# daducci/AMICO

Measured on AMD Instinct MI355X. Metric: voxels/sec (whole node), NODDI fit, higher is better.
Workload: dtype f64; 1 GPU; NODDI fit, 1000000 masked voxels per GPU, 99-volume 2-shell scheme (9 b0 + 30@b700 + 60@b2000), 145 atoms, ndirs=500, inputs resident in HBM; voxels_per_gpu=1000000, global_voxels=1000000, parallelism=voxel shards x1, one RCCL all_gather of the maps per step

## Files before the change

amico_amd/csrc/amx_seed.hpp:

```cpp
#pragma once
#include "amx_kernels.hpp"

namespace amx {

constexpr int kSeedMax = 8;
constexpr int kSeed3ListRow = 36;
constexpr int kSeed3ScanMax = 32;
constexpr int kStageUbNorm = 2;
constexpr int kStageUb = 4;
template <int KD, int LD, int UB = kStageUb>
__device__ __forceinline__ void stage_rows(double *Sl, const double *__restrict__ Sg, int n, int src_ld)
{
    const int N = n * KD;
    for (int e0 = threadIdx.x; e0 < N; e0 += UB * (int)blockDim.x) {
        double v[UB];
#pragma unroll
        for (int u = 0; u < UB; u++) {
            const int e = e0 + u * (int)blockDim.x, ec = e < N ? e : 0, j = ec / KD, d = ec - j * KD;
            v[u] = Sg[(size_t)j * src_ld + d];
        }
#pragma unroll
        for (int u = 0; u < UB; u++) {
            const int e = e0 + u * (int)blockDim.x, j = e / KD, d = e - j * KD;
            if (e < N) Sl[j * LD + d] = v[u];
// ... 74 lines not shown
            int bj = 0; double bn = red[0];
            for (int j = 1; j < n_cols && j < nt; j++) if (red[j] > bn) { bn = red[j]; bj = j; }
            s_j = bj; s_n = bn;
        }
        __syncthreads();
        const double nn = s_n;
        const bool live = nn > 1e-280;
        for (int i = tid; i < nS; i += nt) Q[d * nS + i] = live ? R[i * ldA + s_j] / sqrt(nn) : 0.0;
        __syncthreads();
        for (int pass = 0; pass < 2 && live; pass++) {
            if (tid < d) { double c = 0.0; for (int i = 0; i < nS; i++) c += Q[tid * nS + i] * Q[d * nS + i]; s_coef[tid] = c; }
            __syncthreads();
            for (int i = tid; i < nS; i += nt) { double v = Q[d * nS + i]; for (int e = 0; e < d; e++) v -= s_coef[e] * Q[e * nS + i]; Q[d * nS + i] = v; }
            __syncthreads();
            if (tid == 0) { double c = 0.0; for (int i = 0; i < nS; i++) c += Q[d * nS + i] * Q[d * nS + i]; s_n = c; }
            __syncthreads();
            const double n2 = s_n;
            for (int i = tid; i < nS; i += nt) Q[d * nS + i] = n2 > 0.0 ? Q[d * nS + i] / sqrt(n2) : 0.0;
            __syncthreads();
        }
        if (tid < n_cols) {
            double c = 0.0;
            for (int i = 0; i < nS; i++) c += Q[d * nS + i] * R[i * ldA + tid];
            for (int i = 0; i < nS; i++) R[i * ldA + tid] -= c * Q[d * nS + i];
        }
        __syncthreads();
    }
    if (kap != nullptr) {
        double en = 0.0, an = 0.0;
        if (tid < n_cols) {
            for (int i = 0; i < nS; i++) {
                const double v = R[i * ldA + tid]; en += v * v;
                double o = (rowsel == nullptr || rowsel[i]) ? (double)g[i * ldA + tid] : 0.0;
                if (colscale != nullptr) o *= colscale[tid];
                an += o * o;
            }
        }
        red[tid] = en;
        __syncthreads();
        if (tid == 0) { double m = 0.0; for (int j = 0; j < n_cols && j < nt; j++) m = red[j] > m ? red[j] : m; s_n = m; }
        __syncthreads();
        const double emax = sqrt(s_n);
        __syncthreads();
        red[tid] = an;
        __syncthreads();
        if (tid == 0) { double m = 0.0; for (int j = 0; j < n_cols && j < nt; j++) m = red[j] > m ? red[j] : m; kap[dir] = emax + 2e-6 * sqrt(m); if (kap0) kap0[dir] = emax; }
        __syncthreads();
    }
    double *U = Ub + (size_t)dir * nS * KD;
    for (int e = tid; e < nS * KD; e += nt) { const int i = e / KD, d = e - i * KD; U[e] = Q[d * nS + i]; }
    double *S = Sb + (size_t)dir * n_cols * KD;
    for (int e = tid; e < n_cols * KD; e += nt) {
        const int j = e / KD, d = e - j * KD;
        double c = 0.0;
        for (int i = 0; i < nS; i++) {
            double v = (rowsel == nullptr || rowsel[i]) ? (double)g[i * ldA + j] : 0.0;
            c += Q[d * nS + i] * v;
        }
        if (colscale != nullptr) c *= colscale[j];
        S[e] = c;
        if (Sf != nullptr) Sf[(size_t)dir * KD * kScreenLd + d * kScreenLd + j] = (float)c;
    }
}

struct SeedArgs {
    const double *y;
    const float *y32;
    const int *perm;
    const Chunk *chunks;
    const int *n_chunks;
    const Chunk *schunks;
    const int *n_schunks;
    const double *Ub, *Sb;
    double *ytil;
    unsigned long long *seeds;
    const unsigned long long *cand8; const unsigned char *cdone;
    const unsigned long long *supp;
    int nS, n_atoms, iso_atom, dot_atom;
    int *gcount;
    int n_gcount;
    int *stats;
    int trip_cap;
    int fork_skip;
};

template <int NR>
__global__ void __launch_bounds__(1024) k_noddi_project(const SeedArgs a)
{
    constexpr int KD = kSeedKD;
    const int cid = xcd_chunk((int)blockIdx.x, *a.n_chunks);
    if (cid < 0) return;
    const Chunk ck = a.chunks[cid];
    const int lane = threadIdx.x & 63, wave = threadIdx.x >> 6, nw = (int)blockDim.x >> 6;
    const int nS = a.nS;
    double ur[NR][KD];
    const double *U = a.Ub + (size_t)ck.dir * nS * KD;
#pragma unroll
    for (int rr = 0; rr < NR; rr++) {
        const int i = lane + kWave * rr;
#pragma unroll
        for (int d = 0; d < KD; d++) ur[rr][d] = (i < nS) ? U[i * KD + d] : 0.0;
    }
    for (int k = wave; k < ck.count; k += nw) {
        const int pos = ck.start + k;
        const size_t yo = (size_t)a.perm[pos] * nS;
        double yr[NR];
#pragma unroll
        for (int rr = 0; rr < NR; rr++) { const int i = lane + kWave * rr; yr[rr] = (i < nS) ? (a.y32 ? (double)a.y32[yo + i] : a.y[yo + i]) : 0.0; }
        double out = 0.0;
#pragma unroll
        for (int b = 0; b < KD; b += 4) {
            double p[4];
#pragma unroll
            for (int u = 0; u < 4; u++) {
                p[u] = 0.0;
#pragma unroll
                for (int rr = 0; rr < NR; rr++) p[u] += ur[rr][b + u] * yr[rr];
            }
            wave_sum4(p, lane);
#pragma unroll
            for (int u = 0; u < 4; u++) out = (lane == b + u) ? p[u] : out;
        }
        if (lane < KD) a.ytil[(size_t)pos * KD + lane] = out;
    }
}

__device__ __forceinline__ double seed_div(double x, double d)
{
    double r = __builtin_amdgcn_rcp(d);
    r = r * (2.0 - d * r);
    r = r * (2.0 - d * r);
    const double q = x * r;
    return q + r * (x - q * d);
}

template <int N> __device__ __forceinline__ constexpr int stri(int i, int j) { return i * (i + 1) / 2 + j; }


__device__ __forceinline__ double seed_max(double a, double b)
{
    double d;
    asm("v_max_f64 %0, %1, %2" : "=v"(d) : "v"(a), "v"(b));
    return d;
}

__device__ __forceinline__ double seed_min(double a, double b)
{
    double d;
    asm("v_min_f64 %0, %1, %2" : "=v"(d) : "v"(a), "v"(b));
    return d;
}

typedef double seed_v4d __attribute__((ext_vector_type(4)));
template <int KS, int MT, bool PIPE = true>
__device__ __forceinline__ void seed_scan_mfma(const double *Aop, double *Rb, const double (&r)[4 * KS], int lane, double &best, int &bj)
{
    constexpr int KDP = 4 * KS + 1;
    const int q = lane >> 4, c16 = lane & 15;
#pragma unroll
    for (int d = 0; d < 4 * KS; d++) Rb[lane * KDP + d] = r[d];
    double b[4][KS];
#pragma unroll
    for (int nt = 0; nt < 4; nt++) {
#pragma unroll
        for (int ks = 0; ks < KS; ks++) b[nt][ks] = Rb[(16 * nt + c16) * KDP + 4 * ks + q];
    }
    const double ninf = -__builtin_huge_val();
    double bv[4] = {ninf, ninf, ninf, ninf};
    auto products = [&](int mt, seed_v4d (&acc)[4]) {
        double av[KS];
#pragma unroll
        for (int ks = 0; ks < KS; ks++) av[ks] = Aop[(mt * KS + ks) * 64 + lane];
#pragma unroll
        for (int nt = 0; nt < 4; nt++) acc[nt] = (seed_v4d){0.0, 0.0, 0.0, 0.0};
#pragma unroll
        for (int ks = 0; ks < KS; ks++) {
#pragma unroll
            for (int nt = 0; nt < 4; nt++) acc[nt] = __builtin_amdgcn_mfma_f64_16x16x4f64(av[ks], b[nt][ks], acc[nt], 0, 0, 0);
        }
    };
    seed_v4d cur[4], nxt[PIPE ? 4 : 1];
    if (PIPE) products(0, cur);
#pragma unroll
    for (int mt = 0; mt < MT; mt++) {
        if (PIPE) { if (mt + 1 < MT) products(mt + 1, reinterpret_cast<seed_v4d (&)[4]>(nxt)); }
        else products(mt, cur);
        __builtin_amdgcn_sched_barrier(0);
#pragma unroll
        for (int nt = 0; nt < 4; nt++) {
#pragma unroll
            for (int rr = 0; rr < 4; rr++) {
                const double v = cur[nt][rr];
                const unsigned lo = ((unsigned)__double2loint(v) & 0xffffff00u) | (unsigned)(mt * 4 + rr);
                bv[nt] = seed_max(bv[nt], __hiloint2double(__double2hiint(v), (int)lo));
            }
        }
        __builtin_amdgcn_sched_barrier(0);
        if (PIPE) {
#pragma unroll
            for (int nt = 0; nt < 4; nt++) cur[nt] = nxt[PIPE ? nt : 0];
        }
    }
    double mine = ninf;
#pragma unroll
    for (int nt = 0; nt < 4; nt++) {
        const double t = __hiloint2double(__double2hiint(bv[nt]), (int)((unsigned)__double2loint(bv[nt]) | (unsigned)(q << 6)));
        const double m = rows_allmax(t);
        mine = (q == nt) ? m : mine;
    }
    const unsigned code = (unsigned)__double2loint(mine) & 0xffu;
    best = mine;
    bj = 16 * (int)((code >> 2) & 15u) + 4 * (int)(code & 3u) + (int)(code >> 6);
}

template <int MS>
struct SeedLane {
    static constexpr int NT = MS * (MS + 1) / 2;
    double T[NT], dinv[MS], c[MS], x[MS];
    int idx[MS], np;

    __device__ __forceinline__ void clear()
    {
        np = 0;
#pragma unroll
        for (int s = 0; s < MS; s++) { idx[s] = 0; x[s] = 0.0; c[s] = 0.0; dinv[s] = 0.0; }
#pragma unroll
        for (int e = 0; e < NT; e++) T[e] = 0.0;
    }
    __device__ __forceinline__ void solve(double (&z)[MS]) const
    {
#pragma unroll
        for (int j = 0; j < MS; j++) {
            double f = c[j];
#pragma unroll
            for (int m = 0; m < j; m++) f -= T[stri<MS>(j, m)] * z[m];
            z[j] = f * dinv[j];
        }
#pragma unroll
        for (int j = MS - 1; j >= 0; j--) {
            double f = z[j];
#pragma unroll
            for (int m = j + 1; m < MS; m++) f -= T[stri<MS>(m, j)] * z[m];
            z[j] = f * dinv[j];
        }
    }
    __device__ __forceinline__ void solve_rhs(const double (&b)[MS], double (&z)[MS]) const
    {
#pragma unroll
        for (int j = 0; j < MS; j++) {
            double f = b[j];
#pragma unroll
            for (int m = 0; m < j; m++) f -= T[stri<MS>(j, m)] * z[m];
            z[j] = f * dinv[j];
        }
#pragma unroll
        for (int j = MS - 1; j >= 0; j--) {
            double f = z[j];
#pragma unroll
            for (int m = j + 1; m < MS; m++) f -= T[stri<MS>(m, j)] * z[m];
            z[j] = f * dinv[j];
        }
    }
    __device__ __forceinline__ bool factor()
    {
        bool ok = true;
#pragma unroll
        for (int j = 0; j < MS; j++) {
            double dj = T[stri<MS>(j, j)];
            const double hjj = dj;
#pragma unroll
            for (int m = 0; m < j; m++) dj -= T[stri<MS>(j, m)] * T[stri<MS>(j, m)];
            const bool good = dj > 1e-15 * hjj;
            ok = ok && (j >= np || good);
            dinv[j] = (j < np && good) ? inv_sqrt(dj) : 0.0;
            T[stri<MS>(j, j)] = dj * dinv[j];
#pragma unroll
            for (int i = j + 1; i < MS; i++) {
                double v = T[stri<MS>(i, j)];
#pragma unroll
                for (int m = 0; m < j; m++) v -= T[stri<MS>(i, m)] * T[stri<MS>(j, m)];
                T[stri<MS>(i, j)] = v * dinv[j];
            }
        }
        return ok;
    }
    __device__ __forceinline__ void remove(int k)
    {
        double l[MS];
#pragma unroll
        for (int i = 0; i < MS - 1; i++) {
            double v = 0.0;
#pragma unroll
            for (int kk = 0; kk <= i; kk++) v = (k == kk) ? T[stri<MS>(i + 1, kk)] : v;
            l[i] = v;
        }
        l[MS - 1] = 0.0;
        __builtin_amdgcn_sched_barrier(0);
#pragma unroll
        for (int i = 0; i < MS - 1; i++) {
#pragma unroll
            for (int j = 0; j <= i; j++) {
                const double v00 = T[stri<MS>(i, j)], v10 = T[stri<MS>(i + 1, j)], v11 = T[stri<MS>(i + 1, j + 1)];
                T[stri<MS>(i, j)] = (i < k) ? v00 : ((j < k) ? v10 : v11);
            }
            __builtin_amdgcn_sched_barrier(0);
        }
        __builtin_amdgcn_sched_barrier(0);
#pragma unroll
        for (int m = 0; m < MS; m++) T[stri<MS>(MS - 1, m)] = (k < MS) ? 0.0 : T[stri<MS>(MS - 1, m)];
#pragma unroll
        for (int s = 0; s < MS - 1; s++) {
            const bool mv = s >= k;
            idx[s] = mv ? idx[s + 1] : idx[s]; x[s] = mv ? x[s + 1] : x[s]; c[s] = mv ? c[s + 1] : c[s]; dinv[s] = mv ? dinv[s + 1] : dinv[s];
        }
        if (k < MS) { idx[MS - 1] = 0; x[MS - 1] = 0.0; c[MS - 1] = 0.0; dinv[MS - 1] = 0.0; np -= 1; }
        __builtin_amdgcn_sched_barrier(0);
#pragma unroll
        for (int j = 0; j < MS - 1; j++) {
            const double a = T[stri<MS>(j, j)], b = l[j];
            const bool rot = b != 0.0;
            const double n2 = a * a + b * b;
            const double ri = rot ? inv_sqrt(n2) : dinv[j];
            const double ss = rot ? b * dinv[j] : 0.0;
            const double cc = rot ? n2 * ri * dinv[j] : 1.0;
            const double ci = rot ? a * ri : 1.0;
            T[stri<MS>(j, j)] = rot ? n2 * ri : a;
            dinv[j] = ri;
#pragma unroll
            for (int i = j + 1; i < MS - 1; i++) {
                const double t = (T[stri<MS>(i, j)] + ss * l[i]) * ci;
                l[i] = cc * l[i] - ss * t;
                T[stri<MS>(i, j)] = t;
            }
            __builtin_amdgcn_sched_barrier(0);
        }
    }
    __device__ __forceinline__ int step(const double (&z)[MS])
    {
        double nb = 0.0, db = 1.0;
        int kmin = -1;
#pragma unroll
        for (int s = 0; s < MS; s++) {
            const bool neg = s < np && !(z[s] > 0.0);
            const double den = x[s] - z[s];
            const double num = (den > 0.0) ? x[s] : 0.0, dd = (den > 0.0) ? den : 1.0;
            const bool better = neg && (kmin < 0 || num * db < nb * dd);
            nb = better ? num : nb; db = better ? dd : db; kmin = better ? s : kmin;
        }
        const double alpha = seed_div(nb, db);
#pragma unroll
        for (int s = 0; s < MS; s++) x[s] = (kmin < 0) ? z[s] : ((s < np) ? x[s] + alpha * (z[s] - x[s]) : 0.0);
        return kmin;
    }
};

struct SeedFeed {
    int lo, hi;
    bool more;
    int left;
    __device__ __forceinline__ void reset() { lo = 0; hi = 0; more = true; left = 1 << 30; }
    __device__ __forceinline__ bool pending() const { return more || lo < hi; }
    __device__ __forceinline__ int take(unsigned long long needm, int *gcount, int count, int lane)
// ... 132 lines not shown
                V.clear();
                if (STAGE == 3) {
#pragma unroll
                    for (int q4 = 0; q4 < 4; q4++) allow[STAGE == 3 ? q4 : 0] = nallow[(PREF && STAGE == 3) ? q4 : 0];
                    ncand = -1;
                }
                if (finite) active = true;
                else a.seeds[pos] = kNoSeed;
            }
            const unsigned long long needm = __ballot(!have_next);
            if (needm != 0ull && feed.pending()) {
                const int k = feed.take(needm, a.gcount + cid, ck.count, lane);
                if (k >= 0) {
                    next_pos = ck.start + k; have_next = true;
                    const double *yp = a.ytil + (size_t)next_pos * KD;
#pragma unroll
                    for (int d = 0; d < KD; d++) ynext[PREF ? d : 0] = yp[d];
                    if (STAGE == 3) {
                        const int vox = a.perm[next_pos];
#pragma unroll
                        for (int q4 = 0; q4 < 4; q4++) nallow[(PREF && STAGE == 3) ? q4 : 0] = a.supp[(size_t)vox * 4 + q4];
                        nallow[(PREF && STAGE == 3) ? (a.iso_atom >> 6) : 0] |= 1ull << (a.iso_atom & 63);
                        if (a.dot_atom >= 0) nallow[(PREF && STAGE == 3) ? (a.dot_atom >> 6) : 0] |= 1ull << (a.dot_atom & 63);
                    }
                }
            }
            if (__ballot(active) == 0ull) {
                if (!feed.pending() && __ballot(have_next) == 0ull) break;
                continue;
            }
        } else {
        const unsigned long long freem = __ballot(!active);
        if (freem != 0ull && feed.pending()) {
            const int k = feed.take(freem, a.gcount + cid, ck.count, lane);
            if (k >= 0) {
                pos = ck.start + k;
                bool finite = true;
                trips = 0; last_added = -1; ban0 = -1; ban1 = -1;
                V.clear();
                ncand = -1;
                if (STAGE == 3) {
                    bool ready = false;
                    if (a.cand8 != nullptr) {
                        const unsigned long long *cl = a.cand8 + (size_t)pos * 4;
                        const unsigned long long c0 = cl[0], c1 = cl[1], c2 = cl[2], c3 = cl[3];
                        const int flag = (int)a.cdone[pos];
                        ready = flag == 1;
                        if (ready) { cand[0] = c0; cand[STAGE == 3 ? 1 : 0] = c1; cand[STAGE == 3 ? 2 : 0] = c2; cand[STAGE == 3 ? 3 : 0] = c3 & 0x00ffffffffffffffull; ncand = (int)(c3 >> 56); }
                    }
                    if (a.fork_skip && !ready) { finite = false; ncand = 0; }
                    else if (__ballot(!ready) != 0ull) {
                        if (!ready) {
                            const int vox = a.perm[pos];
#pragma unroll
                            for (int q = 0; q < 4; q++) allow[q] = a.supp[(size_t)vox * 4 + q];
                            allow[a.iso_atom >> 6] |= 1ull << (a.iso_atom & 63);
                            if (a.dot_atom >= 0) allow[a.dot_atom >> 6] |= 1ull << (a.dot_atom & 63);
                        }
                    }
                }
                if (finite) active = true;
                else a.seeds[pos] = (STAGE == 3 && a.fork_skip) ? kSeedForked : kNoSeed;
            }
        }
        if (__ballot(active) == 0ull) {
            if (!feed.pending()) break;
            continue;
        }
        }
        if (STAGE == 3) {
            if (__ballot(ncand < 0) != 0ull) {
                const bool fresh = ncand < 0;
                unsigned char *row = reinterpret_cast<unsigned char *>(ticket + 4) + (size_t)threadIdx.x * kSeed3ListRow;
                if (fresh) {
#pragma unroll
                    for (int w8 = 0; w8 < 8; w8++) reinterpret_cast<unsigned *>(row)[w8] = 0u;
                }
                int nc = 0;
#pragma unroll
                for (int q = 0; q < 4; q++) {
                    unsigned long long rem = fresh ? allow[q] : 0ull;
                    for (int it = 0; it < 64; it++) {
                        if (__ballot(rem != 0ull) == 0ull) break;
                        if (rem != 0ull) {
                            const int j = q * 64 + __builtin_ctzll(rem);
                            rem &= rem - 1ull;
                            if (nc < 32) row[nc] = (unsigned char)j;
                            nc++;
                        }
                    }
                }
                if (fresh) {
#pragma unroll
                    for (int w4 = 0; w4 < 4; w4++) {
                        const unsigned lo = reinterpret_cast<const unsigned *>(row)[2 * w4], hi = reinterpret_cast<const unsigned *>(row)[2 * w4 + 1];
                        cand[STAGE == 3 ? w4 : 0] = ((unsigned long long)hi << 32) | (unsigned long long)lo;
                    }
                    ncand = nc;
                    if (nc > 32 && active) { a.seeds[pos] = kNoSeed; active = false; }
                }
            }
        }
#ifdef AMX_STATS
        st_trips++; st_used += __builtin_popcountll(__ballot(active));
#endif
        trips++;
        SEED_PH(0);
        bool scan = active;
        {
            double z[MS];
            V.solve(z);
            int kmin = V.step(z);
            if (active && kmin < 0) { ban0 = -1; ban1 = -1; }
            if (__ballot(active && kmin >= 0) != 0ull) {
                bool ok = true;
                if (active && kmin >= 0) {
                    int gone = 0;
#pragma unroll
                    for (int s = 0; s < MS; s++) gone = (s == kmin) ? V.idx[s] : gone;
                    if (gone == last_added) { ban1 = ban0; ban0 = gone; }
                }
                __builtin_amdgcn_sched_barrier(0);
                V.remove((active && kmin >= 0) ? kmin : MS);
                __builtin_amdgcn_sched_barrier(0);
                V.solve(z);
                if (active && kmin >= 0) {
                    if (!ok) scan = false;
                    else if (V.step(z) >= 0) scan = false;
                }
            }
        }
        SEED_PH(1);
        bool done = false;
        bool noseed = false;
        if (__ballot(scan) != 0ull) {
            const double *yp = a.ytil + (size_t)pos * KD;
            double r[KD];
#pragma unroll
            for (int d = 0; d < KD; d++) r[d] = PREF ? yv[PREF ? d : 0] : yp[d];
#pragma unroll
            for (int s = 0; s < MS; s++) {
                const double *col = Sl + V.idx[s] * LD;
                double cv[KD];
                seed_col<KD>(col, cv);
#pragma unroll
                for (int d = 0; d < KD; d++) r[d] -= V.x[s] * cv[d];
            }
            SEED_PH(2);
            const bool rfin = fabs(r[0]) <= 1.79769313486231570e308;
            double best = -inf;
            int bj = -1;
            if (STAGE == 1) {
                if (n_atoms <= 16 * MT) {
                    seed_scan_mfma<KS, MT, (!OCC2 && kSeed1Occ == 1)>(Aop, Rb, r, lane, best, bj);
                } else {
                    for (int j = 0; j < n_atoms; j++) {
                        const double *sp = Sg + (size_t)j * KD;
                        double w = 0.0;
#pragma unroll
                        for (int d = 0; d < KD; d++) w += sp[d] * r[d];
                        const bool ok = w > best;
                        best = ok ? w : best; bj = ok ? j : bj;
                    }
                }
                if (__ballot(scan && (bj == ban0 || bj == ban1)) != 0ull) {
#ifdef AMX_STATS
                    ph[5] += 1024;
#endif
                    best = -inf; bj = -1;
                    for (int j = 0; j < n_atoms; j++) {
                        const double *sp = Sg + (size_t)j * KD;
                        double w = 0.0;
#pragma unroll
                        for (int d = 0; d < KD; d++) w += sp[d] * r[d];
                        const bool ok = (j != ban0) && (j != ban1) && (w > best);
                        best = ok ? w : best; bj = ok ? j : bj;
                    }
                }
            } else {
#pragma unroll
                for (int it = 0; it < kSeed3ScanMax; it += 2) {
                    if (__ballot(scan && it < ncand) == 0ull) break;
                    const int j0 = (int)((cand[STAGE == 3 ? (it >> 3) : 0] >> (8 * (it & 7))) & 0xffull);
                    const int j1 = (int)((cand[STAGE == 3 ? ((it + 1) >> 3) : 0] >> (8 * ((it + 1) & 7))) & 0xffull);
                    const double2 *c0 = reinterpret_cast<const double2 *>(Sl + j0 * LD), *c1 = reinterpret_cast<const double2 *>(Sl + j1 * LD);
                    double u0[KD], u1[KD];
#pragma unroll
                    for (int d = 0; d < KD; d += 2) {
                        const double2 p0 = c0[d >> 1], p1 = c1[d >> 1];
                        u0[d] = p0.x; u0[d + 1] = p0.y; u1[d] = p1.x; u1[d + 1] = p1.y;
                    }
                    double w0a = 0.0, w0b = 0.0, w1a = 0.0, w1b = 0.0;
#pragma unroll
                    for (int d = 0; d < KD; d += 2) { w0a += u0[d] * r[d]; w0b += u0[d + 1] * r[d + 1]; w1a += u1[d] * r[d]; w1b += u1[d + 1] * r[d + 1]; }
                    const double w0 = w0a + w0b, w1 = w1a + w1b;
                    const bool ok0 = scan && (it < ncand) && (j0 != ban0) && (j0 != ban1) && (w0 > best) && !(iso_first && V.np == 0 && j0 == a.iso_atom);
                    best = ok0 ? w0 : best; bj = ok0 ? j0 : bj;
                    const bool ok1 = scan && (it + 1 < ncand) && (j1 != ban0) && (j1 != ban1) && (w1 > best) && !(iso_first && V.np == 0 && j1 == a.iso_atom);
                    best = ok1 ? w1 : best; bj = ok1 ? j1 : bj;
                }
                if (iso_first && __ballot(scan && V.np == 0 && !(best > tol)) != 0ull) {
                    const double *ci = Sl + a.iso_atom * LD;
                    double si[KD], wi = 0.0;
                    seed_col<KD>(ci, si);
#pragma unroll
                    for (int d = 0; d < KD; d++) wi += si[d] * r[d];
                    const bool oki = scan && V.np == 0 && !(best > tol) && wi > best;
                    best = oki ? wi : best; bj = oki ? a.iso_atom : bj;
                }
            }
            SEED_PH(3);
            if (scan) {
                bool inp = false;
#pragma unroll
                for (int s = 0; s < MS; s++) inp = inp || (s < V.np && V.idx[s] == bj);
                if (!rfin) {
                    done = true; noseed = true; V.np = 0;
                } else if (!(best > tol) || bj < 0 || inp) {
                    done = true;
                } else if (V.np >= MS || trips > trip_cap) {
                    done = true; noseed = true;
                } else {
                    if (iso_first) {
                        const double *ci = Sl + a.iso_atom * LD;
                        double si[KD], ciso = 0.0, hii = 0.0;
                        seed_col<KD>(ci, si);
#pragma unroll
                        for (int d = 0; d < KD; d++) { ciso += si[d] * (PREF ? yv[PREF ? d : 0] : yp[d]); hii += si[d] * si[d]; }
                        const bool pre = V.np == 0 && bj != a.iso_atom && ciso > tol && hii > 0.0;
                        const double di0 = pre ? inv_sqrt(hii) : 0.0;
                        V.T[stri<MS>(0, 0)] = pre ? hii * di0 : V.T[stri<MS>(0, 0)];
                        V.dinv[0] = pre ? di0 : V.dinv[0];
                        V.idx[0] = pre ? a.iso_atom : V.idx[0];
                        V.c[0] = pre ? ciso : V.c[0];
                        V.x[0] = pre ? 0.0 : V.x[0];
                        V.np += pre ? 1 : 0;
                    }
                    const double *ct = Sl + bj * LD;
                    double st[KD], cn = 0.0, htt = 0.0;
                    seed_col<KD>(ct, st);
#pragma unroll
                    for (int d = 0; d < KD; d++) { cn += st[d] * (PREF ? yv[PREF ? d : 0] : yp[d]); htt += st[d] * st[d]; }
                    double h[MS];
#pragma unroll
                    for (int s = 0; s < MS; s++) {
                        const double *col = Sl + V.idx[s] * LD;
                        double cv[KD];
                        seed_col<KD>(col, cv);
                        double v = 0.0;
#pragma unroll
                        for (int d = 0; d < KD; d++) v += cv[d] * st[d];
                        h[s] = (s < V.np) ? v : 0.0;
                    }
                    double dd = htt;
#pragma unroll
                    for (int j = 0; j < MS; j++) {
                        double f = h[j];
#pragma unroll
                        for (int m = 0; m < j; m++) f -= V.T[stri<MS>(j, m)] * h[m];
                        h[j] = f * V.dinv[j];
                        dd -= h[j] * h[j];
                    }
                    const bool good = dd > 1e-15 * htt;
                    const double di = good ? inv_sqrt(dd) : 0.0;
                    if (!good) {
                        ban1 = ban0; ban0 = bj;
                    } else {
#pragma unroll
                        for (int i = 0; i < MS; i++) {
                            const bool here = (V.np == i);
#pragma unroll
                            for (int j = 0; j < i; j++) V.T[stri<MS>(i, j)] = here ? h[j] : V.T[stri<MS>(i, j)];
                            V.T[stri<MS>(i, i)] = here ? dd * di : V.T[stri<MS>(i, i)];
                            V.dinv[i] = here ? di : V.dinv[i];
                            V.idx[i] = here ? bj : V.idx[i]; V.c[i] = here ? cn : V.c[i]; V.x[i] = here ? 0.0 : V.x[i];
                        }
                        last_added = bj;
                        V.np += 1;
                    }
                }
            }
        }
        SEED_PH(4);
        if (active && !done && trips > 2 * trip_cap) { done = true; noseed = true; }
        if (done) {
            unsigned lo = 0xffffffffu, hi = 0xffffffffu;
            if (!noseed || (STAGE == 1 && V.np > 0)) {
#pragma unroll
                for (int s = 0; s < 4; s++) {
                    if (s < V.np) lo = (lo & ~(0xffu << (8 * s))) | ((unsigned)(V.idx[s] & 0xff) << (8 * s));
                    if (s + 4 < V.np && s + 4 < MS) hi = (hi & ~(0xffu << (8 * s))) | ((unsigned)(V.idx[s + 4 < MS ? s + 4 : 0] & 0xff) << (8 * s));
                }
                if (V.np == 0) lo = 0xfffffffeu;
            }
            a.seeds[pos] = ((unsigned long long)hi << 32) | (unsigned long long)lo;
            active = false;
        }
#ifdef AMX_STATS
        pt = (long long)__builtin_readcyclecounter();
#endif
    }
    __syncthreads();
    }
#ifdef AMX_STATS
    if (a.stats && lane == 0) {
        atomicAdd(&a.stats[0], st_trips); atomicAdd(&a.stats[1], st_used);
        if (STAGE == 1) for (int k = 0; k < 6; k++) atomicAdd(&a.stats[8 + k], (int)(ph[k] >> 10));
// ... 1067 lines not shown
                double g = on ? (clip ? 1.0 : st) * (ct - sub - xq * giso[tc]) - lam1 : -1.0;
#pragma unroll
                for (int s = 0; s < MS; s++) { const double xv = (s < V.np && on) ? xs[s] : 0.0; g -= st * gv[s] * xv; }
                if (on && !(g < -1e-10)) viol = true;
                n_ex += on ? 1 : 0;
            }
        }
        GC_PH(3);
        const bool cert = good && !viol;
        if (valid) a.done[pos] = cert ? 1 : 0;
        if (WIDE && a.qcount != nullptr) {
            const unsigned long long qm = __ballot(valid && !cert && flag == 0ull && cnt > MS && cnt <= a.q_hi);
            if (qm != 0ull && lane == 0) atomicAdd(&a.qcount[cid], __builtin_popcountll(qm));
        }
        {
            const unsigned long long rm = __ballot(valid && !cert);
            if (rm != 0ull) {
                int base = 0;
                if (lane == 0) base = atomicAdd(&a.rcount[cid], __builtin_popcountll(rm));
                base = __builtin_amdgcn_readfirstlane(base);
                const int rank = __builtin_amdgcn_mbcnt_hi((unsigned)(rm >> 32), __builtin_amdgcn_mbcnt_lo((unsigned)rm, 0u));
                if (valid && !cert) a.rlist[ck.start + base + rank] = pos;
            }
        }
#ifdef AMX_STATS
        if (a.stats) {
            const int nc = __builtin_popcountll(__ballot(cert)), nv = __builtin_popcountll(__ballot(valid));
            const int nbig = __builtin_popcountll(__ballot(valid && flag == 0ull && cnt > MS)), nfe = __builtin_popcountll(__ballot(valid && okv && piv && !feas)), nvi = __builtin_popcountll(__ballot(valid && good && viol));
            if (lane == 0) { atomicAdd(&a.stats[0], nv); atomicAdd(&a.stats[1], nc); atomicAdd(&a.stats[2], nbig); atomicAdd(&a.stats[3], nfe); atomicAdd(&a.stats[4], nvi); }
            int ne = n_ex;
            for (int o = 32; o > 0; o >>= 1) ne += __shfl_xor(ne, o);
            if (lane == 0) atomicAdd(&a.stats[5], ne);
        }
#endif
        if (cert) {
            unsigned long long *sp = a.supp + (size_t)vox * 4;
            sp[0] = Pq[0]; sp[1] = Pq[1]; sp[2] = Pq[2]; sp[3] = 0ull;
            if (a.cand8 != nullptr) {
                static_assert(MS + 2 <= 31, "the list is 31 bytes and its length");
                const int n_extra = a.dot_atom >= 0 ? 2 : 1;
                const int e0 = a.dot_atom >= 0 ? a.dot_atom : a.iso_atom, e1 = a.iso_atom;
                unsigned long long w[4] = {wl[0], wl[1], wl[2], wl[3]};
#pragma unroll
                for (int s = 1; s < MS + 2; s++) {
                    const int b = (s == V.np ? e0 : ((s == V.np + 1 && n_extra == 2) ? e1 : 0));
                    w[s >> 3] |= (unsigned long long)(b & 0xff) << (8 * (s & 7));
                }
                if (V.np == 0) w[0] |= (unsigned long long)(e0 & 0xff);
                w[3] = (w[3] & 0x00ffffffffffffffull) | ((unsigned long long)(V.np + n_extra) << 56);
                unsigned long long *cl = a.cand8 + (size_t)pos * 4;
                cl[0] = w[0]; cl[1] = w[1]; cl[2] = w[2]; cl[3] = w[3];
            }
            if (a.xdbg) {
                double *dst = a.xdbg + ((size_t)vox * 3 + 1) * a.n_atoms;
                for (int j = 0; j < a.n_atoms; j++) dst[j] = 0.0;
#pragma unroll
                for (int s = 0; s < MS; s++) if (s < V.np) dst[V.idx[s]] = V.c[s];
                dst[a.iso_atom] = xi;
                if (a.dot_atom >= 0) dst[a.dot_atom] = a.xiso[(size_t)vox * 2 + 1];
            }
        }
        GC_PH(4);
    }
    __syncthreads();
    }
#ifdef AMX_STATS
    if (!WIDE && a.stats && lane == 0) for (int q5 = 0; q5 < 5; q5++) atomicAdd(&a.stats[34 + q5], (int)(gph[q5] >> 10));
#endif
}

constexpr int kSeed2KD = 8;
constexpr int kSeed2Ld = kSeedKD;
struct Seed2Args {
    const double *y;
    const float *y32;
    const int *perm;
    const Chunk *chunks;
    const int *n_chunks;
    const Chunk *schunks;
    const int *n_schunks;
    const float *tiles;
    int tile_stride, ldA;
    const unsigned char *rowdwi;
    const double *xiso;
    const double *Ub, *Sb;
    double *ytil;
    unsigned long long *seeds;
    int nS, n_wm, iso_atom, is_exvivo;
    double lam1, lam2;
    int *gcount;
    int n_gcount;
    int *stats;
    double *trace;
    int trip_cap;
    int max_atoms;
};

template <int NR>
__global__ void __launch_bounds__(1024) k_noddi_project2(const Seed2Args a)
{
    constexpr int KD = kSeed2Ld;
    const int cid = xcd_chunk((int)blockIdx.x, *a.n_chunks);
    if (cid < 0) return;
    const Chunk ck = a.chunks[cid];
    const int lane = threadIdx.x & 63, wave = threadIdx.x >> 6, nw = (int)blockDim.x >> 6;
    const int nS = a.nS;
    double ur[NR][KD], isov[NR];
    bool rowok[NR];
    const double *U = a.Ub + (size_t)ck.dir * nS * KD;
    const float *tile = a.tiles + (size_t)ck.dir * a.tile_stride;
#pragma unroll
    for (int rr = 0; rr < NR; rr++) {
        const int i = lane + kWave * rr;
        rowok[rr] = (i < nS) && a.rowdwi[i];
        isov[rr] = (i < nS) ? (double)tile[i * a.ldA + a.iso_atom] : 0.0;
#pragma unroll
        for (int d = 0; d < KD; d++) ur[rr][d] = (i < nS) ? U[i * KD + d] : 0.0;
    }
    for (int k = wave; k < ck.count; k += nw) {
        const int pos = ck.start + k;
        const int vox = a.perm[pos];
        const size_t yo = (size_t)vox * nS;
        const double xi = a.xiso[(size_t)vox * 2], xd = a.xiso[(size_t)vox * 2 + 1];
        double yr[NR];
#pragma unroll
        for (int rr = 0; rr < NR; rr++) {
            const int i = lane + kWave * rr;
            double t = 0.0;
            if (rowok[rr]) {
                t = (a.y32 ? (double)a.y32[yo + i] : a.y[yo + i]) - xi * isov[rr];
                if (a.is_exvivo) t -= xd * 1.0;
                if (t < 0.0) t = 0.0;
            }
            yr[rr] = t;
        }
        double out = 0.0;
#pragma unroll
        for (int b = 0; b < KD; b += 4) {
            double p[4];
#pragma unroll
            for (int u = 0; u < 4; u++) {
                p[u] = 0.0;
#pragma unroll
                for (int rr = 0; rr < NR; rr++) p[u] += ur[rr][b + u] * yr[rr];
            }
            wave_sum4(p, lane);
#pragma unroll
            for (int u = 0; u < 4; u++) out = (lane == b + u) ? p[u] : out;
        }
        if (lane < KD) a.ytil[(size_t)pos * KD + lane] = out;
    }
}

constexpr int kSeed2Occ = 1;
template <bool OCC2 = false>
__global__ void __launch_bounds__(256, OCC2 ? 2 : kSeed2Occ) k_lasso_seed(const Seed2Args a)
{
    constexpr int KD = kSeed2KD, KS = KD / 4, MT = 9, KDP = KD + 1, NT = KD * (KD + 1) / 2, LD = KD + 1;
    extern __shared__ __attribute__((aligned(16))) unsigned char smem_l[];
    double *Sl = reinterpret_cast<double *>(smem_l);
    const int n_wm = a.n_wm;
    unsigned *ticket = reinterpret_cast<unsigned *>(Sl + (size_t)n_wm * LD);
    double *Aop = reinterpret_cast<double *>(ticket + 4);
    double *Rb = Aop + MT * KS * 64 + (threadIdx.x >> 6) * (64 * KDP + 64 * 3);
    unsigned long long *Pb = reinterpret_cast<unsigned long long *>(Rb + 64 * KDP);
    const int n_sch = *a.n_schunks;
    const int own = xcd_chunk((int)blockIdx.x, n_sch);
    if (own < 0) return;
    const int lane = threadIdx.x & 63, q = lane >> 4, c16 = lane & 15;
    constexpr int SLD = kSeed2Ld;
#ifdef AMX_STATS
    int st_trips = 0, st_used = 0;
#endif
    for (int round = 0; round < 256; round++) {
    const int cid = seed_next_chunk(round, own, a.schunks, n_sch, a.gcount, a.gcount + a.n_gcount, reinterpret_cast<int *>(ticket), 32 * (int)(blockDim.x >> 6));
    if (cid < 0) break;
    const Chunk ck = a.schunks[cid];
    const double *__restrict__ Sg = a.Sb + (size_t)ck.dir * n_wm * SLD;
    stage_rows<KD, LD>(Sl, Sg, n_wm, SLD);
    stage_operand<KS, MT>(Aop, Sg, n_wm, SLD);
    __syncthreads();
    const double lam1 = a.lam1, lam2 = a.lam2, tol = 1e-9, inf = __builtin_huge_val();
    const double sl2 = sqrt(lam2), isl2 = 1.0 / sl2;
    const int trip_cap = a.trip_cap;

    bool active = false;
    int pos = 0, trips = 0;
    double T[NT], dinv[KD], g[KD];
    unsigned long long P[3] = {0ull, 0ull, 0ull};
#pragma unroll
    for (int e = 0; e < NT; e++) T[e] = 0.0;
#pragma unroll
    for (int d = 0; d < KD; d++) { dinv[d] = 0.0; g[d] = 0.0; }
    SeedFeed feed;
    feed.reset();
    constexpr bool PREF2 = !OCC2 && kSeed2Occ == 1;
    double yv[KD], ynext[PREF2 ? KD : 1];
    int next_pos = -1;
    bool have_next = false;
    for (int guard = 0; guard < (1 << 20); ++guard) {
        if (PREF2) {
        if (!active && have_next) {
            pos = next_pos; have_next = false;
            bool finite = true;
#pragma unroll
            for (int d = 0; d < KD; d++) { yv[d] = ynext[PREF2 ? d : 0]; finite = finite && (fabs(yv[d]) <= 1.79769313486231570e308); }
            trips = 0;
            P[0] = 0ull; P[1] = 0ull; P[2] = 0ull;
#pragma unroll
            for (int i = 0; i < KD; i++) {
#pragma unroll
                for (int j = 0; j <= i; j++) T[stri<KD>(i, j)] = (i == j) ? sl2 : 0.0;
                dinv[i] = isl2; g[i] = 0.0;
            }
            if (finite) active = true;
            else { a.seeds[(size_t)pos * 4 + 3] = ~0ull; }
        }
        {
            const unsigned long long needm = __ballot(!have_next);
            if (needm != 0ull && feed.pending()) {
                const int k = feed.take(needm, a.gcount + cid, ck.count, lane);
                if (k >= 0) {
                    next_pos = ck.start + k; have_next = true;
                    const double *yp = a.ytil + (size_t)next_pos * SLD;
#pragma unroll
                    for (int d = 0; d < KD; d++) ynext[PREF2 ? d : 0] = yp[d];
                }
            }
        }
        if (__ballot(active) == 0ull) {
            if (!feed.pending() && __ballot(have_next) == 0ull) break;
            continue;
        }
        } else {
            const unsigned long long freem = __ballot(!active);
            if (freem != 0ull && feed.pending()) {
                const int k = feed.take(freem, a.gcount + cid, ck.count, lane);
                if (k >= 0) {
                    pos = ck.start + k;
                    const double *yp = a.ytil + (size_t)pos * SLD;
                    bool finite = true;
#pragma unroll
                    for (int d = 0; d < KD; d++) { yv[d] = yp[d]; finite = finite && (fabs(yv[d]) <= 1.79769313486231570e308); }
                    trips = 0;
                    P[0] = 0ull; P[1] = 0ull; P[2] = 0ull;
#pragma unroll
                    for (int i = 0; i < KD; i++) {
#pragma unroll
                        for (int j = 0; j <= i; j++) T[stri<KD>(i, j)] = (i == j) ? sl2 : 0.0;
                        dinv[i] = isl2; g[i] = 0.0;
                    }
                    if (finite) active = true;
                    else { a.seeds[(size_t)pos * 4 + 3] = ~0ull; }
                }
            }
            if (__ballot(active) == 0ull) {
                if (!feed.pending()) break;
                continue;
            }
        }
#ifdef AMX_STATS
        st_trips++; st_used += __builtin_popcountll(__ballot(active));
#endif
        trips++;
        double r[KD];
        {
            double w[KD];
#pragma unroll
            for (int j = 0; j < KD; j++) {
                double f = g[j];
#pragma unroll
                for (int m = 0; m < j; m++) f -= T[stri<KD>(j, m)] * w[m];
                w[j] = f * dinv[j];
            }
#pragma unroll
            for (int j = KD - 1; j >= 0; j--) {
                double f = w[j];
#pragma unroll
                for (int m = j + 1; m < KD; m++) f -= T[stri<KD>(m, j)] * w[m];
                w[j] = f * dinv[j];
            }
#pragma unroll
            for (int d = 0; d < KD; d++) r[d] = yv[d] - w[d];
        }
        int dj = -1;
        double best = -inf, best2 = -inf;
        int bj = -1, bj2 = -1;
        {
#pragma unroll
            for (int d = 0; d < KD; d++) Rb[lane * KDP + d] = r[d];
#pragma unroll
            for (int w3 = 0; w3 < 3; w3++) Pb[lane * 3 + w3] = active ? P[w3] : ~0ull;
            double b[4][KS];
#pragma unroll
            for (int nt = 0; nt < 4; nt++) {
#pragma unroll
                for (int ks = 0; ks < KS; ks++) b[nt][ks] = Rb[(16 * nt + c16) * KDP + 4 * ks + q];
            }
            const double ninf = -inf;
            double bv[4] = {ninf, ninf, ninf, ninf};
            double wv[4] = {ninf, ninf, ninf, ninf};
            double b2[4] = {ninf, ninf, ninf, ninf};
            auto products = [&](int mt, seed_v4d (&acc)[4]) {
                double av[KS];
#pragma unroll
                for (int ks = 0; ks < KS; ks++) av[ks] = Aop[(mt * KS + ks) * 64 + lane];
#pragma unroll
                for (int nt = 0; nt < 4; nt++) acc[nt] = (seed_v4d){0.0, 0.0, 0.0, 0.0};
#pragma unroll
                for (int ks = 0; ks < KS; ks++) {
#pragma unroll
                    for (int nt = 0; nt < 4; nt++) acc[nt] = __builtin_amdgcn_mfma_f64_16x16x4f64(av[ks], b[nt][ks], acc[nt], 0, 0, 0);
                }
            };
            seed_v4d cur[4], nxt[PREF2 ? 4 : 1];
            if (PREF2) products(0, cur);
#pragma unroll
            for (int mt = 0; mt < MT; mt++) {
                if (PREF2) { if (mt + 1 < MT) products(mt + 1, reinterpret_cast<seed_v4d (&)[4]>(nxt)); }
                else products(mt, cur);
                unsigned long long pw[4];
#pragma unroll
                for (int nt = 0; nt < 4; nt++) pw[nt] = Pb[(16 * nt + c16) * 3 + ((16 * mt) >> 6)] >> q;
                __builtin_amdgcn_sched_barrier(0);
#pragma unroll
                for (int nt = 0; nt < 4; nt++) {
#pragma unroll
                    for (int rr = 0; rr < 4; rr++) {
                        const int bit = 16 * mt + 4 * rr;
                        const bool pas = (pw[nt] >> (bit & 63)) & 1ull;
                        const double v = cur[nt][rr];
                        const unsigned lo = ((unsigned)__double2loint(v) & 0xffffff00u) | (unsigned)(mt * 4 + rr);
                        const int hi = pas ? (int)0xffe00000 : __double2hiint(v);
                        const double val = __hiloint2double(hi, (int)lo);
                        b2[nt] = seed_max(b2[nt], seed_min(bv[nt], val));
                        bv[nt] = seed_max(bv[nt], val);
                        const int hn = pas ? (__double2hiint(v) ^ (int)0x80000000) : (int)0xffe00000;
                        wv[nt] = seed_max(wv[nt], __hiloint2double(hn, (int)lo));
                    }
                }
                __builtin_amdgcn_sched_barrier(0);
                if (PREF2) {
#pragma unroll
                    for (int nt = 0; nt < 4; nt++) cur[nt] = nxt[PREF2 ? nt : 0];
                }
            }
            double mine = ninf;
#pragma unroll
            for (int nt = 0; nt < 4; nt++) {
                const double t = __hiloint2double(__double2hiint(bv[nt]), (int)((unsigned)__double2loint(bv[nt]) | (unsigned)(q << 6)));
                const double m = rows_allmax(t);
                mine = (q == nt) ? m : mine;
            }
            const unsigned code = (unsigned)__double2loint(mine) & 0xffu;
            best = mine - lam1;
            bj = 16 * (int)((code >> 2) & 15u) + 4 * (int)(code & 3u) + (int)(code >> 6);
            double second = ninf;
#pragma unroll
            for (int nt = 0; nt < 4; nt++) {
                const double t1 = __hiloint2double(__double2hiint(bv[nt]), (int)((unsigned)__double2loint(bv[nt]) | (unsigned)(q << 6)));
                const double t2 = __hiloint2double(__double2hiint(b2[nt]), (int)((unsigned)__double2loint(b2[nt]) | (unsigned)(q << 6)));
                const double mall = rows_allmax(t1);
                const double m = rows_allmax((t1 == mall) ? t2 : t1);
                second = (q == nt) ? m : second;
            }
            const unsigned codes = (unsigned)__double2loint(second) & 0xffu;
            best2 = second - lam1;
            bj2 = 16 * (int)((codes >> 2) & 15u) + 4 * (int)(codes & 3u) + (int)(codes >> 6);
            double mine2 = ninf;
#pragma unroll
            for (int nt = 0; nt < 4; nt++) {
                const double t = __hiloint2double(__double2hiint(wv[nt]), (int)((unsigned)__double2loint(wv[nt]) | (unsigned)(q << 6)));
                const double m = rows_allmax(t);
                mine2 = (q == nt) ? m : mine2;
            }
            const unsigned code2 = (unsigned)__double2loint(mine2) & 0xffu;
            if (active && mine2 > -1e300 && -mine2 - lam1 <= 0.0)
                dj = 16 * (int)((code2 >> 2) & 15u) + 4 * (int)(code2 & 3u) + (int)(code2 >> 6);
        }
        bool done = false, noseed = false;
        int jj = -1, jj2 = -1;
        double sigma = 0.0, sigma2 = 0.0;
        if (active) {
            const int cnt = __builtin_popcountll(P[0]) + __builtin_popcountll(P[1]) + __builtin_popcountll(P[2]);
            const bool add1 = best > tol && bj < n_wm, add2 = best2 > tol && bj2 < n_wm;
            const int mx = a.max_atoms;
            if (dj >= 0) { jj = dj; sigma = -1.0; if (add1 && cnt < mx) { jj2 = bj; sigma2 = 1.0; } }
            else if (add1) { jj = bj; sigma = 1.0; if (add2 && cnt < mx - 1) { jj2 = bj2; sigma2 = 1.0; } }
            else done = true;
            if (!done && (trips > trip_cap || (sigma > 0.0 && cnt >= mx))) { done = true; noseed = true; jj = -1; sigma = 0.0; jj2 = -1; sigma2 = 0.0; }
        }
#pragma unroll 1
        for (int ch = 0; ch < 2; ch++) {
            const int jc = ch == 0 ? jj : jj2;
            const double sg = ch == 0 ? sigma : sigma2;
            if (ch == 1 && __ballot(jc >= 0) == 0ull) break;
            double v[KD];
            const double *col = Sl + (jc >= 0 ? jc : 0) * LD;
            double cj = -lam1;
#pragma unroll
            for (int d = 0; d < KD; d++) { v[d] = (jc >= 0) ? col[d] : 0.0; cj += v[d] * yv[d]; }
#pragma unroll
            for (int d = 0; d < KD; d++) g[d] += sg * cj * v[d];
            if (jc >= 0) P[jc >> 6] ^= 1ull << (jc & 63);
#pragma unroll
            for (int j = 0; j < KD; j++) {
                const double al = T[stri<KD>(j, j)], bl = v[j];
                const bool rot = bl != 0.0;
                const double n2 = al * al + sg * bl * bl;
                const double ri = rot ? ((n2 > 0.0) ? inv_sqrt(n2) : 0.0) : dinv[j];
                const double ss = rot ? bl * dinv[j] : 0.0;
                const double cc = rot ? n2 * ri * dinv[j] : 1.0;
                const double ci = rot ? al * ri : 1.0;
                T[stri<KD>(j, j)] = rot ? n2 * ri : al;
                dinv[j] = ri;
#pragma unroll
                for (int i = j + 1; i < KD; i++) {
                    const double t = (T[stri<KD>(i, j)] + sg * ss * v[i]) * ci;
                    v[i] = cc * v[i] - ss * t;
                    T[stri<KD>(i, j)] = t;
                }
            }
        }
        if (done) {
            unsigned long long *sd = a.seeds + (size_t)pos * 4;
            sd[0] = P[0]; sd[1] = P[1]; sd[2] = P[2]; sd[3] = noseed ? ~0ull : 0ull;
            active = false;
        }
    }
    __syncthreads();
    }
#ifdef AMX_STATS
    if (a.stats && lane == 0) { atomicAdd(&a.stats[0], st_trips); atomicAdd(&a.stats[1], st_used); }
#endif
}

}
```

Measured before the change: 157.3 million voxels/s.

## Compact active lanes before MFMA atom scan to skip idle 16-lane groups

Before the MFMA-based correlation scan in both seed kernels, lanes that still need work are compacted with ballot/mbcnt into contiguous slots. The residual (and passive mask) is written to those slots, and a templated scan runs only ceil(active/16) MFMA column groups. Results are routed back to each lane with ds_bpermute. This skips MFMA and reduction work for finished voxels in partially active wavefronts. The cost is a switch over four template instances, which adds code size and register pressure, plus the bpermute shuffles.

```diff
diff --git a/amico_amd/csrc/amx_seed.hpp b/amico_amd/csrc/amx_seed.hpp
--- a/amico_amd/csrc/amx_seed.hpp
+++ b/amico_amd/csrc/amx_seed.hpp
@@ -250,42 +250,59 @@
 }
 
 typedef double seed_v4d __attribute__((ext_vector_type(4)));
-template <int KS, int MT, bool PIPE = true>
-__device__ __forceinline__ void seed_scan_mfma(const double *Aop, double *Rb, const double (&r)[4 * KS], int lane, double &best, int &bj)
+
+struct ScanSlots {
+    int cnt, groups, slot;
+    __device__ __forceinline__ ScanSlots(bool need)
+    {
+        const unsigned long long m = __ballot(need);
+        cnt = __builtin_popcountll(m);
+        groups = (cnt + 15) >> 4;
+        slot = (int)__builtin_amdgcn_mbcnt_hi((unsigned)(m >> 32), __builtin_amdgcn_mbcnt_lo((unsigned)m, 0u));
+    }
+    __device__ __forceinline__ double fetch(double v) const
+    {
+        const int lo = __builtin_amdgcn_ds_bpermute(slot << 2, __double2loint(v)), hi = __builtin_amdgcn_ds_bpermute(slot << 2, __double2hiint(v));
+        return __hiloint2double(hi, lo);
+    }
+};
+
+template <int KS, int MT, bool PIPE, int GN>
+__device__ __forceinline__ double seed_scan_groups(const double *Aop, const double *Rb, int lane)
 {
     constexpr int KDP = 4 * KS + 1;
     const int q = lane >> 4, c16 = lane & 15;
-#pragma unroll
-    for (int d = 0; d < 4 * KS; d++) Rb[lane * KDP + d] = r[d];
-    double b[4][KS];
-#pragma unroll
-    for (int nt = 0; nt < 4; nt++) {
+    double b[GN][KS];
+#pragma unroll
+    for (int nt = 0; nt < GN; nt++) {
 #pragma unroll
         for (int ks = 0; ks < KS; ks++) b[nt][ks] = Rb[(16 * nt + c16) * KDP + 4 * ks + q];
     }
     const double ninf = -__builtin_huge_val();
-    double bv[4] = {ninf, ninf, ninf, ninf};
-    auto products = [&](int mt, seed_v4d (&acc)[4]) {
+    double bv[GN];
+#pragma unroll
+    for (int nt = 0; nt < GN; nt++) bv[nt] = ninf;
+    auto products = [&](int mt, seed_v4d (&acc)[GN]) {
         double av[KS];
 #pragma unroll
         for (int ks = 0; ks < KS; ks++) av[ks] = Aop[(mt * KS + ks) * 64 + lane];
 #pragma unroll
-        for (int nt = 0; nt < 4; nt++) acc[nt] = (seed_v4d){0.0, 0.0, 0.0, 0.0};
+        for (int nt = 0; nt < GN; nt++) acc[nt] = (seed_v4d){0.0, 0.0, 0.0, 0.0};
 #pragma unroll
         for (int ks = 0; ks < KS; ks++) {
 #pragma unroll
-            for (int nt = 0; nt < 4; nt++) acc[nt] = __builtin_amdgcn_mfma_f64_16x16x4f64(av[ks], b[nt][ks], acc[nt], 0, 0, 0);
+            for (int nt = 0; nt < GN; nt++) acc[nt] = __builtin_amdgcn_mfma_f64_16x16x4f64(av[ks], b[nt][ks], acc[nt], 0, 0, 0);
         }
     };
-    seed_v4d cur[4], nxt[PIPE ? 4 : 1];
+    seed_v4d cur[GN], nxt[PIPE ? GN : 1];
     if (PIPE) products(0, cur);
 #pragma unroll
     for (int mt = 0; mt < MT; mt++) {
-        if (PIPE) { if (mt + 1 < MT) products(mt + 1, reinterpret_cast<seed_v4d (&)[4]>(nxt)); }
+        if (PIPE) { if (mt + 1 < MT) products(mt + 1, reinterpret_cast<seed_v4d (&)[GN]>(nxt)); }
         else products(mt, cur);
         __builtin_amdgcn_sched_barrier(0);
 #pragma unroll
-        for (int nt = 0; nt < 4; nt++) {
+        for (int nt = 0; nt < GN; nt++) {
 #pragma unroll
             for (int rr = 0; rr < 4; rr++) {
                 const double v = cur[nt][rr];
@@ -296,16 +313,36 @@
         __builtin_amdgcn_sched_barrier(0);
         if (PIPE) {
 #pragma unroll
-            for (int nt = 0; nt < 4; nt++) cur[nt] = nxt[PIPE ? nt : 0];
+            for (int nt = 0; nt < GN; nt++) cur[nt] = nxt[PIPE ? nt : 0];
         }
     }
     double mine = ninf;
 #pragma unroll
-    for (int nt = 0; nt < 4; nt++) {
+    for (int nt = 0; nt < GN; nt++) {
         const double t = __hiloint2double(__double2hiint(bv[nt]), (int)((unsigned)__double2loint(bv[nt]) | (unsigned)(q << 6)));
         const double m = rows_allmax(t);
         mine = (q == nt) ? m : mine;
     }
+    return mine;
+}
+
+template <int KS, int MT, bool PIPE = true>
+__device__ __forceinline__ void seed_scan_mfma(const double *Aop, double *Rb, const double (&r)[4 * KS], int lane, bool need, double &best, int &bj)
+{
+    constexpr int KDP = 4 * KS + 1;
+    const ScanSlots sl(need);
+    if (need) {
+#pragma unroll
+        for (int d = 0; d < 4 * KS; d++) Rb[sl.slot * KDP + d] = r[d];
+    }
+    double mine;
+    switch (sl.groups) {
+    case 1: mine = seed_scan_groups<KS, MT, PIPE, 1>(Aop, Rb, lane); break;
+    case 2: mine = seed_scan_groups<KS, MT, PIPE, 2>(Aop, Rb, lane); break;
+    case 3: mine = seed_scan_groups<KS, MT, PIPE, 3>(Aop, Rb, lane); break;
+    default: mine = seed_scan_groups<KS, MT, PIPE, 4>(Aop, Rb, lane); break;
+    }
+    mine = sl.fetch(mine);
     const unsigned code = (unsigned)__double2loint(mine) & 0xffu;
     best = mine;
     bj = 16 * (int)((code >> 2) & 15u) + 4 * (int)(code & 3u) + (int)(code >> 6);
@@ -744,7 +781,7 @@
             int bj = -1;
             if (STAGE == 1) {
                 if (n_atoms <= 16 * MT) {
-                    seed_scan_mfma<KS, MT, (!OCC2 && kSeed1Occ == 1)>(Aop, Rb, r, lane, best, bj);
+                    seed_scan_mfma<KS, MT, (!OCC2 && kSeed1Occ == 1)>(Aop, Rb, r, lane, scan, best, bj);
                 } else {
                     for (int j = 0; j < n_atoms; j++) {
                         const double *sp = Sg + (size_t)j * KD;
@@ -2118,6 +2155,90 @@
     }
 }
 
+template <int KS, int MT, bool PIPE, int GN>
+__device__ __forceinline__ void lasso_scan_groups(const double *Aop, const double *Rb, const unsigned long long *Pb, int lane, double &mine, double &second, double &mine2)
+{
+    constexpr int KDP = 4 * KS + 1;
+    const int q = lane >> 4, c16 = lane & 15;
+    double b[GN][KS];
+#pragma unroll
+    for (int nt = 0; nt < GN; nt++) {
+#pragma unroll
+        for (int ks = 0; ks < KS; ks++) b[nt][ks] = Rb[(16 * nt + c16) * KDP + 4 * ks + q];
+    }
+    const double ninf = -__builtin_huge_val();
+    double bv[GN], wv[GN], b2[GN];
+#pragma unroll
+    for (int nt = 0; nt < GN; nt++) { bv[nt] = ninf; wv[nt] = ninf; b2[nt] = ninf; }
+    auto products = [&](int mt, seed_v4d (&acc)[GN]) {
+        double av[KS];
+#pragma unroll
+        for (int ks = 0; ks < KS; ks++) av[ks] = Aop[(mt * KS + ks) * 64 + lane];
+#pragma unroll
+        for (int nt = 0; nt < GN; nt++) acc[nt] = (seed_v4d){0.0, 0.0, 0.0, 0.0};
+#pragma unroll
+        for (int ks = 0; ks < KS; ks++) {
+#pragma unroll
+            for (int nt = 0; nt < GN; nt++) acc[nt] = __builtin_amdgcn_mfma_f64_16x16x4f64(av[ks], b[nt][ks], acc[nt], 0, 0, 0);
+        }
+    };
+    seed_v4d cur[GN], nxt[PIPE ? GN : 1];
+    if (PIPE) products(0, cur);
+#pragma unroll
+    for (int mt = 0; mt < MT; mt++) {
+        if (PIPE) { if (mt + 1 < MT) products(mt + 1, reinterpret_cast<seed_v4d (&)[GN]>(nxt)); }
+        else products(mt, cur);
+        unsigned long long pw[GN];
+#pragma unroll
+        for (int nt = 0; nt < GN; nt++) pw[nt] = Pb[(16 * nt + c16) * 3 + ((16 * mt) >> 6)] >> q;
+        __builtin_amdgcn_sched_barrier(0);
+#pragma unroll
+        for (int nt = 0; nt < GN; nt++) {
+#pragma unroll
+            for (int rr = 0; rr < 4; rr++) {
+                const int bit = 16 * mt + 4 * rr;
+                const bool pas = (pw[nt] >> (bit & 63)) & 1ull;
+                const double v = cur[nt][rr];
+                const unsigned lo = ((unsigned)__double2loint(v) & 0xffffff00u) | (unsigned)(mt * 4 + rr);
+                const int hi = pas ? (int)0xffe00000 : __double2hiint(v);
+                const double val = __hiloint2double(hi, (int)lo);
+                b2[nt] = seed_max(b2[nt], seed_min(bv[nt], val));
+                bv[nt] = seed_max(bv[nt], val);
+                const int hn = pas ? (__double2hiint(v) ^ (int)0x80000000) : (int)0xffe00000;
+                wv[nt] = seed_max(wv[nt], __hiloint2double(hn, (int)lo));
+            }
+        }
+        __builtin_amdgcn_sched_barrier(0);
+        if (PIPE) {
+#pragma unroll
+            for (int nt = 0; nt < GN; nt++) cur[nt] = nxt[PIPE ? nt : 0];
+        }
+    }
+    mine = ninf;
+#pragma unroll
+    for (int nt = 0; nt < GN; nt++) {
+        const double t = __hiloint2double(__double2hiint(bv[nt]), (int)((unsigned)__double2loint(bv[nt]) | (unsigned)(q << 6)));
+        const double m = rows_allmax(t);
+        mine = (q == nt) ? m : mine;
+    }
+    second = ninf;
+#pragma unroll
+    for (int nt = 0; nt < GN; nt++) {
+        const double t1 = __hiloint2double(__double2hiint(bv[nt]), (int)((unsigned)__double2loint(bv[nt]) | (unsigned)(q << 6)));
+        const double t2 = __hiloint2double(__double2hiint(b2[nt]), (int)((unsigned)__double2loint(b2[nt]) | (unsigned)(q << 6)));
+        const double mall = rows_allmax(t1);
+        const double m = rows_allmax((t1 == mall) ? t2 : t1);
+        second = (q == nt) ? m : second;
+    }
+    mine2 = ninf;
+#pragma unroll
+    for (int nt = 0; nt < GN; nt++) {
+        const double t = __hiloint2double(__double2hiint(wv[nt]), (int)((unsigned)__double2loint(wv[nt]) | (unsigned)(q << 6)));
+        const double m = rows_allmax(t);
+        mine2 = (q == nt) ? m : mine2;
+    }
+}
+
 constexpr int kSeed2Occ = 1;
 template <bool OCC2 = false>
 __global__ void __launch_bounds__(256, OCC2 ? 2 : kSeed2Occ) k_lasso_seed(const Seed2Args a)
@@ -2253,93 +2374,27 @@
         double best = -inf, best2 = -inf;
         int bj = -1, bj2 = -1;
         {
-#pragma unroll
-            for (int d = 0; d < KD; d++) Rb[lane * KDP + d] = r[d];
-#pragma unroll
-            for (int w3 = 0; w3 < 3; w3++) Pb[lane * 3 + w3] = active ? P[w3] : ~0ull;
-            double b[4][KS];
-#pragma unroll
-            for (int nt = 0; nt < 4; nt++) {
-#pragma unroll
-                for (int ks = 0; ks < KS; ks++) b[nt][ks] = Rb[(16 * nt + c16) * KDP + 4 * ks + q];
-            }
-            const double ninf = -inf;
-            double bv[4] = {ninf, ninf, ninf, ninf};
-            double wv[4] = {ninf, ninf, ninf, ninf};
-            double b2[4] = {ninf, ninf, ninf, ninf};
-            auto products = [&](int mt, seed_v4d (&acc)[4]) {
-                double av[KS];
-#pragma unroll
-                for (int ks = 0; ks < KS; ks++) av[ks] = Aop[(mt * KS + ks) * 64 + lane];
-#pragma unroll
-                for (int nt = 0; nt < 4; nt++) acc[nt] = (seed_v4d){0.0, 0.0, 0.0, 0.0};
-#pragma unroll
-                for (int ks = 0; ks < KS; ks++) {
-#pragma unroll
-                    for (int nt = 0; nt < 4; nt++) acc[nt] = __builtin_amdgcn_mfma_f64_16x16x4f64(av[ks], b[nt][ks], acc[nt], 0, 0, 0);
-                }
-            };
-            seed_v4d cur[4], nxt[PREF2 ? 4 : 1];
-            if (PREF2) products(0, cur);
-#pragma unroll
-            for (int mt = 0; mt < MT; mt++) {
-                if (PREF2) { if (mt + 1 < MT) products(mt + 1, reinterpret_cast<seed_v4d (&)[4]>(nxt)); }
-                else products(mt, cur);
-                unsigned long long pw[4];
-#pragma unroll
-                for (int nt = 0; nt < 4; nt++) pw[nt] = Pb[(16 * nt + c16) * 3 + ((16 * mt) >> 6)] >> q;
-                __builtin_amdgcn_sched_barrier(0);
-#pragma unroll
-                for (int nt = 0; nt < 4; nt++) {
-#pragma unroll
-                    for (int rr = 0; rr < 4; rr++) {
-                        const int bit = 16 * mt + 4 * rr;
-                        const bool pas = (pw[nt] >> (bit & 63)) & 1ull;
-                        const double v = cur[nt][rr];
-                        const unsigned lo = ((unsigned)__double2loint(v) & 0xffffff00u) | (unsigned)(mt * 4 + rr);
-                        const int hi = pas ? (int)0xffe00000 : __double2hiint(v);
-                        const double val = __hiloint2double(hi, (int)lo);
-                        b2[nt] = seed_max(b2[nt], seed_min(bv[nt], val));
-                        bv[nt] = seed_max(bv[nt], val);
-                        const int hn = pas ? (__double2hiint(v) ^ (int)0x80000000) : (int)0xffe00000;
-                        wv[nt] = seed_max(wv[nt], __hiloint2double(hn, (int)lo));
-                    }
-                }
-                __builtin_amdgcn_sched_barrier(0);
-                if (PREF2) {
-#pragma unroll
-                    for (int nt = 0; nt < 4; nt++) cur[nt] = nxt[PREF2 ? nt : 0];
-                }
-            }
-            double mine = ninf;
-#pragma unroll
-            for (int nt = 0; nt < 4; nt++) {
-                const double t = __hiloint2double(__double2hiint(bv[nt]), (int)((unsigned)__double2loint(bv[nt]) | (unsigned)(q << 6)));
-                const double m = rows_allmax(t);
-                mine = (q == nt) ? m : mine;
-            }
+            const ScanSlots sl(active);
+            if (active) {
+#pragma unroll
+                for (int d = 0; d < KD; d++) Rb[sl.slot * KDP + d] = r[d];
+#pragma unroll
+                for (int w3 = 0; w3 < 3; w3++) Pb[sl.slot * 3 + w3] = P[w3];
+            }
+            double mine, second, mine2;
+            switch (sl.groups) {
+            case 1: lasso_scan_groups<KS, MT, PREF2, 1>(Aop, Rb, Pb, lane, mine, second, mine2); break;
+            case 2: lasso_scan_groups<KS, MT, PREF2, 2>(Aop, Rb, Pb, lane, mine, second, mine2); break;
+            case 3: lasso_scan_groups<KS, MT, PREF2, 3>(Aop, Rb, Pb, lane, mine, second, mine2); break;
+            default: lasso_scan_groups<KS, MT, PREF2, 4>(Aop, Rb, Pb, lane, mine, second, mine2); break;
+            }
+            mine = sl.fetch(mine); second = sl.fetch(second); mine2 = sl.fetch(mine2);
             const unsigned code = (unsigned)__double2loint(mine) & 0xffu;
             best = mine - lam1;
             bj = 16 * (int)((code >> 2) & 15u) + 4 * (int)(code & 3u) + (int)(code >> 6);
-            double second = ninf;
-#pragma unroll
-            for (int nt = 0; nt < 4; nt++) {
-                const double t1 = __hiloint2double(__double2hiint(bv[nt]), (int)((unsigned)__double2loint(bv[nt]) | (unsigned)(q << 6)));
-                const double t2 = __hiloint2double(__double2hiint(b2[nt]), (int)((unsigned)__double2loint(b2[nt]) | (unsigned)(q << 6)));
-                const double mall = rows_allmax(t1);
-                const double m = rows_allmax((t1 == mall) ? t2 : t1);
-                second = (q == nt) ? m : second;
-            }
             const unsigned codes = (unsigned)__double2loint(second) & 0xffu;
             best2 = second - lam1;
             bj2 = 16 * (int)((codes >> 2) & 15u) + 4 * (int)(codes & 3u) + (int)(codes >> 6);
-            double mine2 = ninf;
-#pragma unroll
-            for (int nt = 0; nt < 4; nt++) {
-                const double t = __hiloint2double(__double2hiint(wv[nt]), (int)((unsigned)__double2loint(wv[nt]) | (unsigned)(q << 6)));
-                const double m = rows_allmax(t);
-                mine2 = (q == nt) ? m : mine2;
-            }
             const unsigned code2 = (unsigned)__double2loint(mine2) & 0xffu;
             if (active && mine2 > -1e300 && -mine2 - lam1 <= 0.0)
                 dj = 16 * (int)((code2 >> 2) & 15u) + 4 * (int)(code2 & 3u) + (int)(code2 >> 6);
```

Measured after the change: 163.0 million voxels/s, median of 6. 3.6% higher.
